# bcgsc/abyss

Hardware: AMD Instinct MI355X
Metric: Mk-mers/s inserted+extended (abyss-bloom-dbg, k=64); unitig bit-exact (higher is better)
Workload: dtype u64

## Files before the change

### abyss_amd/csrc/abg_core.h

```cpp
#pragma once

#include <stdint.h>
#include <stddef.h>

#if defined(__HIPCC__)
#include <hip/hip_runtime.h>
#define ABG_HD __host__ __device__ __forceinline__
#define ABG_HDN __host__ __device__
#define ABG_HDX __host__ __device__ __attribute__((noinline))
#else
#define ABG_HD inline
#define ABG_HDN
#define ABG_HDX
#endif

namespace abg {

constexpr int MAX_NW = 6;
constexpr int MAX_HASHES = 32;
constexpr unsigned FP_TRIM = 5;

enum Dir : int { FORWARD = 0, REVERSE = 1 };
enum Sense : int { SENSE = 0, ANTISENSE = 1 };

// ... 588 lines not shown
		rh[j] = srol_back(Q[j + k - 1] ^ (j ? Q[j - 1] : 0), j);
	}
}
#if defined(__HIP_DEVICE_COMPILE__)
ABG_HD uint64_t shfl64(uint64_t v, unsigned src)
{
	return ((uint64_t)(uint32_t)__shfl((int)(v >> 32), (int)src) << 32) | (uint32_t)__shfl((int)(uint32_t)v, (int)src);
}
template <int NW>
ABG_HD void stretch_hashes_wave(const uint32_t* __restrict__ words, uint64_t woff, uint32_t qlo, uint32_t n, unsigned k,
    uint64_t& fh, uint64_t& rh)
{
	const unsigned lane = __lane_id();
	const uint32_t nb = n + k - 1;
	const uint32_t epl = (nb + 63) >> 6;
	uint64_t pf[STRETCH_EPL], pr[STRETCH_EPL];
	uint64_t af = 0, ar = 0;
	const uint32_t t0 = lane * epl, bp0 = qlo + t0;
	uint64_t two = 0;
	if (t0 < nb) {
		const uint32_t tl = t0 + epl - 1u < nb ? t0 + epl - 1u : nb - 1u;
		const uint64_t wi = woff + (bp0 >> 4);
		const uint32_t lo = words[wi];
		const uint32_t hi = ((qlo + tl) >> 4) != (bp0 >> 4) ? words[wi + 1] : 0u;
		two = (uint64_t)lo | ((uint64_t)hi << 32);
	}
#pragma unroll
	for (unsigned i = 0; i < STRETCH_EPL; i++) {
		const uint32_t t = t0 + i;
		if (i < epl && t < nb) {
			const unsigned base = (unsigned)(two >> (2u * ((bp0 & 15u) + i))) & 3u;
			af ^= srol_back(seed_of(base), t); ar ^= srol_fwd(seed_of(3u - base), t);
		}
		pf[i] = af; pr[i] = ar;
	}
	uint64_t sf = af, sr = ar;
#pragma unroll
	for (unsigned d = 1; d < 64; d <<= 1) {
		const uint64_t tf = shfl64(sf, lane >= d ? lane - d : lane), tr = shfl64(sr, lane >= d ? lane - d : lane);
		if (lane >= d) { sf ^= tf; sr ^= tr; }
	}
	sf ^= af; sr ^= ar;
#pragma unroll
	for (unsigned i = 0; i < STRETCH_EPL; i++) { pf[i] ^= sf; pr[i] ^= sr; }
	auto fetch = [&](uint32_t t, uint64_t& vf, uint64_t& vr) {
		const unsigned src = t / epl, idx = t - src * epl;
		vf = 0; vr = 0;
#pragma unroll
		for (unsigned i = 0; i < STRETCH_EPL; i++) {
			if (i >= epl) break;
			const uint64_t xf = shfl64(pf[i], src & 63u), xr = shfl64(pr[i], src & 63u);
			if (idx == i) { vf = xf; vr = xr; }
		}
	};
	const uint32_t l = lane < n ? lane : 0;
	uint64_t hf, hr, lf, lr;
	fetch(l + k - 1, hf, hr);
	fetch(l ? l - 1 : 0, lf, lr);
	if (!l) { lf = 0; lr = 0; }
	fh = srol_fwd(hf ^ lf, k - 1 + l);
	rh = srol_back(hr ^ lr, l);
}
#endif

template <int NW, class Get>
ABG_HD Vtx<NW> gather_vertex(const Params& p, bool coop, Get get)
// ... 1499 lines not shown
```

### abyss_amd/csrc/abg_engine.h

```cpp
#pragma once
#include "abg_walk.h"

#include <algorithm>
#include <chrono>
#include <cstdio>
#include <cstdlib>
#include <cstring>
#include <functional>
#include <future>
#include <string>
#include <type_traits>
#include <vector>

namespace abg {

struct Failure { int code; std::string msg; };
constexpr int FAIL_INVAL = -1, FAIL_NOMEM = -3, FAIL_INTERNAL = -4;
[[noreturn]] inline void fail_now(int code, const std::string& msg) { throw Failure{ code, msg }; }
inline std::string strf(const char* fmt, unsigned long long a = 0, unsigned long long b = 0)
{
	char buf[256];
	snprintf(buf, sizeof buf, fmt, a, b);
	return buf;
}
// ... 18 lines not shown
	uint32_t cosettle_passes = 6;
	uint32_t cosettle_log2 = 24;
	uint32_t walk_slots = 4096;
	uint32_t tb_cap = 512;
	uint32_t buf_cap = 1u << 16;
	uint64_t pool_cap = 1ull << 28;
	uint32_t rec_cap = 1u << 22;
	uint32_t wtab_log2 = 26;
	uint32_t wtab_log2_max = 31;
	uint32_t cend_log2 = 20;
	uint64_t p2_first_batch = 65536;
	uint64_t p2_max_batch = 1ull << 22;
	uint32_t p2_growth = 2;
	uint32_t p2_crowded = 1u << 18;
	uint32_t p2_starved_growth = 2;
	uint32_t p2_starved = 6144;
	uint32_t slice_filter = 0;
	bool solid_plane = true;
	uint32_t classify_slots = 65536;
	uint32_t cls_both_max_mb = 1024;
	bool cls_both = true;
	bool prefetch_classify = true;
	uint32_t memo_log2 = 0;
	bool memo = true;
	uint32_t p2_max_candidates = 1u << 18;
	uint32_t t_tags = 1024;
	uint32_t commit_incremental = 1;
	uint32_t commit_dirty_max = 4096;
	uint32_t commit_dirty_log2 = 26;
	uint32_t guide_stride = 4;
	uint32_t guide_log2_max = 31;
	bool guide_seen = true;
	bool link_duplicates = true;
	bool par_commit = true;
	bool overlap_bins = true;
	bool overlap_purity = true;
	uint32_t dist_hash_all_ranks = 2;
	uint32_t dist_route_min_ranks = 4;
	uint64_t keep_insert_scratch_bytes = 16ull << 30;
	uint64_t par_commit_max_bytes = 16ull << 30;
	int verbose = 0;
};

struct Counters {
	uint64_t solid_reads = 0, visited_reads = 0, reads_processed = 0, bases_assembled = 0,
	         contig_id = 0;
};

struct BaseCodes {
	uint8_t t[256];
	BaseCodes()
	{
		for (int i = 0; i < 256; i++) t[i] = 0xFF;
		t['A'] = t['a'] = 0; t['C'] = t['c'] = 1; t['G'] = t['g'] = 2; t['T'] = t['t'] = 3;
	}
};
template <class T>
struct NoInitAlloc : std::allocator<T> {
	template <class U> struct rebind { using other = NoInitAlloc<U>; };
	template <class U, class... A> void construct(U* p, A&&... a)
	{
		if constexpr (sizeof...(A) == 0) ::new ((void*)p) U; else ::new ((void*)p) U(std::forward<A>(a)...);
	}
};
struct HostBatch {
	std::vector<uint32_t, NoInitAlloc<uint32_t>> words;
// ... 1605 lines not shown
		env->fast = (char*)fast + a;
		env->fast_bytes = fast_bytes - a;
		env->coop = coop;
		walk_read<NW>(*env, list[i], slot);
	}
};

template <int NW>
ABG_HDN uint64_t seq_kmer_hash(const Params& p, const uint8_t* seq, uint64_t j)
{
	return scratch_hash(p, [&](unsigned i) { return (unsigned)seq[j + i]; });
}
template <int NW>
ABG_HDN uint64_t read_kmer_hash(const Params& p, const Batch& b, uint64_t r, uint32_t j)
{
	return scratch_hash(p, [&](unsigned i) { return batch_base(b, r, j + i); });
}
constexpr uint32_t PREP_RUN = 8;
ABG_HD uint64_t dup_mix(uint64_t x) { x ^= x >> 31; x *= 0xD6E8FEB86659FD93ULL; x ^= x >> 29; x *= 0x9E3779B97F4A7C15ULL; x ^= x >> 32; return x | 1; }
template <int NW>
struct FReadPrep {
	Params p; Batch b; const uint32_t* cand_read; const uint64_t* rkoff; uint64_t* rkh; uint32_t first;
	ABG_HDN void operator()(uint64_t i, uint32_t lane, uint32_t nlanes) const
	{
		uint32_t c = first + (uint32_t)i;
		uint64_t r = cand_read[c];
		uint32_t nk = b.len[r] - p.k + 1;
		uint64_t* out = rkh + rkoff[c];
		for (uint32_t j0 = lane * PREP_RUN; j0 < nk; j0 += nlanes * PREP_RUN)
			kmer_hash_run(p, [&](unsigned q) { return batch_base(b, r, q); }, j0, j0 + PREP_RUN < nk ? j0 + PREP_RUN : nk,
			    [&](uint32_t j, uint64_t h) { out[j] = h; });
	}
};
template <int NW>
struct FContigPrep {
	Params p; const uint8_t* cnt; ContigRec* recs; uint32_t first; const uint8_t* pool; uint64_t* kh;
	uint32_t with_cov;
	ABG_HDN void operator()(uint64_t i, uint32_t lane, uint32_t nlanes) const
	{
		ContigRec& rec = recs[first + i];
		const uint8_t* seq = pool + rec.seq_off;
		uint64_t* out = kh + rec.seq_off;
		uint32_t cnk = rec.len - p.k + 1;
		uint32_t cov = 0;
		uint64_t fp = 0;
		for (uint32_t j0 = lane * PREP_RUN; j0 < cnk; j0 += nlanes * PREP_RUN)
			kmer_hash_run(p, [&](unsigned q) { return (unsigned)seq[q]; }, j0, j0 + PREP_RUN < cnk ? j0 + PREP_RUN : cnk,
			    [&](uint32_t j, uint64_t h) { out[j] = h; fp += dup_mix(h); if (with_cov) cov += solid_min_count(p, cnt, h); });
		if (cov) atomic_add_u32(&rec.coverage, cov);
		if (fp) atomic_add_u64(&rec.fp, fp);
	}
};

struct FDupKeys {
	const ContigRec* recs; uint32_t k; uint64_t* key; uint32_t* val;
	ABG_HD void operator()(uint64_t i, uint32_t) const
	{
		const ContigRec& r = recs[i];
		key[i] = r.len < k + FP_TRIM - 1 ? ~0ULL - i : dup_mix(r.fp ^ ((uint64_t)r.len << 40));
		val[i] = (uint32_t)i;
	}
};
struct FDupLink {
	ContigRec* recs; const uint64_t* key; const uint32_t* val; uint64_t n; uint32_t first_new;
	ABG_HD void operator()(uint64_t q, uint32_t) const
	{
		const uint32_t me = val[q];
		if (me < first_new) return;
		const uint64_t k = key[q];
		uint64_t g = q;
		for (unsigned s = 0; s < 64 && g > 0 && key[g - 1] == k; s++) g--;
		uint32_t best = REC_END, best_cand = recs[me].cand;
		for (unsigned s = 0; s < 128 && g < n && key[g] == k; s++, g++) {
			const uint32_t o = val[g];
			if (o != me && recs[o].cand < best_cand && recs[o].len == recs[me].len && recs[o].fp == recs[me].fp) { best = o; best_cand = recs[o].cand; }
		}
		recs[me].dup_of = best;
	}
};
struct FDupVerify {
	ContigRec* recs; const uint64_t* kh; uint32_t k; uint32_t first_new;
// ... 459 lines not shown
		if (!stop) c = c0 + nchunk;
	}
	if (tid == 0) e.st->break_at = c;
	sy.barrier();
}

constexpr uint32_t T_NEVER = 0xFFFFFFFFu;
constexpr uint32_t T_TIME_BITS = 22, T_TAGS = 1u << (32 - T_TIME_BITS);
ABG_HD uint32_t t_stamp(uint32_t tag, uint32_t time) { return (tag << T_TIME_BITS) | time; }
ABG_HD uint32_t t_read(uint32_t v, uint32_t tag) { return (v >> T_TIME_BITS) == tag ? (v & ((1u << T_TIME_BITS) - 1)) : T_NEVER; }
struct ParCommit {
	Params p; Batch b;
	const uint32_t* cand_read; const uint32_t* status; const uint32_t* first_rec;
	ContigRec* recs; const uint8_t* pool; uint8_t* result;
	const uint64_t* kh; const uint64_t* rkh; const uint64_t* rkoff; const uint8_t* read_flag;
	const uint8_t* cnt8;
	uint32_t* vis32;
	uint32_t* both32 = nullptr;
	ContigArchive arc{};
	uint32_t* T;
	uint64_t* Tk;
	uint32_t* Tv;
	uint64_t Tmask;
	uint32_t tag;
	WalkTab cend;
	WalkTab tcend;
	uint32_t* off;
	uint32_t* cnt;
	uint32_t* cnt2;
	uint64_t* cnt3;
	uint8_t* active;
	uint32_t* short_list;
	VKey* short_keys;
	uint32_t* scal;
	uint32_t* nfirst;
	uint32_t* dirty; uint32_t dirty_cap;
	uint32_t* A; uint32_t A_shift;
	uint32_t c_begin, c_end, brk;
	uint64_t own_lo, own_span;
	uint8_t* part_c; uint8_t* part_r;
};
constexpr uint64_t T_KEY_EMPTY = ~0ULL;
ABG_HD uint64_t pc_T_hash(const ParCommit& e, uint64_t pos)
{
	uint64_t x = pos * 0x9E3779B97F4A7C15ULL;
	x ^= x >> 32;
	return x & e.Tmask;
}
ABG_HD uint32_t* pc_T_slot(const ParCommit& e, uint64_t pos)
{
	if (e.T) return &e.T[pos];
	uint64_t s = pc_T_hash(e, pos);
	for (;;) {
		const uint64_t cur = cas_u64(&e.Tk[s], T_KEY_EMPTY, pos);
		if (cur == T_KEY_EMPTY || cur == pos) return &e.Tv[s];
		s = (s + 1) & e.Tmask;
	}
}
ABG_HD uint32_t pc_T_get(const ParCommit& e, uint64_t pos)
{
	if (e.T) return e.T[pos];
	uint64_t s = pc_T_hash(e, pos);
	for (;;) {
		const uint64_t cur = e.Tk[s];
		if (cur == pos) return e.Tv[s];
		if (cur == T_KEY_EMPTY) return T_NEVER;
// ... 113 lines not shown
			if (!rec.ins) continue;
			const uint64_t* ch = e.kh + rec.seq_off;
			const uint32_t cnk = rec.len - e.p.k + 1;
			for (uint32_t j = lane; j < cnk; j += nlanes) {
				uint64_t h = ch[j];
				const uint32_t which = inc ? pc_dirty_mask(e, h) : ~0u;
				if (!which) continue;
				for (unsigned q = 0; q < e.p.nh; q++) {
					if (!((which >> q) & 1u)) continue;
					const uint64_t pos = pos_i(e.p, h, q);
					if (pos - e.own_lo < e.own_span) atomic_min_u32(pc_T_slot(e, pos), t_stamp(e.tag, rec.time));
				}
			}
		}
	}
};
ABG_HD void wt_upsert_min(const WalkTab& t, const VKey& key, uint64_t time)
{
	uint64_t s = wt_slot(t, key, 0);
	for (uint64_t probes = 0; probes <= t.mask; probes++, s = (s + 1) & t.mask) {
		uint64_t cur = t.hmin[s];
		if (cur == WT_EMPTY) { t.hmin[s] = key.fh; t.hmax[s] = key.rh; t.meta[s] = time; return; }
		if (cur == key.fh && t.hmax[s] == key.rh) { if (time < t.meta[s]) t.meta[s] = time; return; }
	}
}
struct FPcShortKeys {
	ParCommit e;
	ABG_HDN void operator()(uint64_t i, uint32_t) const
	{
		const ContigRec& rec = e.recs[e.short_list[i]];
		const uint8_t* seq = e.pool + rec.seq_off;
		e.short_keys[2 * i] = canonical_end_key(e.p, seq);
		e.short_keys[2 * i + 1] = canonical_end_key(e.p, seq + rec.len - e.p.k);
	}
};
struct FPcShort {
	ParCommit e; uint32_t mode;
	ABG_HDN void operator()(uint64_t, uint32_t) const
	{
		const uint32_t n = e.scal[2];
		uint32_t added = 0;
		for (uint32_t i = 0; i < n; i++) {
			const ContigRec& rec = e.recs[e.short_list[i]];
			if (!rec.ins) continue;
			if (mode == 1 && rec.cand >= e.brk) continue;
			const VKey k1 = e.short_keys[2 * i], k2 = e.short_keys[2 * i + 1];
			if (mode == 0) {
				wt_upsert_min(e.tcend, k1, rec.time);
				wt_upsert_min(e.tcend, k2, rec.time);
			} else {
				int a = wt_insert(e.cend, k1, 0, 0), b = wt_insert(e.cend, k2, 0, 0);
				added += (a == WT_NEW) + (b == WT_NEW);
				if (a == WT_FULL || b == WT_FULL) e.scal[4] = 1;
			}
		}
		if (mode == 1) e.scal[3] = added;
	}
};
ABG_HD bool pc_end_before(const ParCommit& e, const VKey& key, uint32_t time)
{
	if (wt_find(e.cend, key, 0) != WT_EMPTY) return true;
	uint64_t s = wt_find(e.tcend, key, 0);
	return s != WT_EMPTY && e.tcend.meta[s] < (uint64_t)time;
}
template <class E>
ABG_HD bool pc_owns_no_unset_bit(const E& e, const ContigRec& rec, uint32_t lane, uint32_t nlanes, bool owned_only)
// ... 1759 lines not shown
		e.nfirst = nfirst;
		const bool incremental = cfg_.commit_incremental && (cfg_.commit_incremental > 1 || !t_hashed()) && !part && cfg_.commit_dirty_max > 0 && nrec > 0;
		uint32_t* dirty_buf = nullptr;
		e.dirty = nullptr; e.dirty_cap = 0; e.A = nullptr; e.A_shift = 0;
		if (incremental) {
			e.dirty_cap = (uint32_t)std::min<uint64_t>(std::min(cfg_.commit_dirty_max, 8192u), std::max(nrec, 1u));
			dirty_buf = (uint32_t*)be_.alloc(2ull * e.dirty_cap * 4 + 8);
			e.dirty = dirty_buf;
			if (!pcA_) {
				const uint32_t log2 = std::min(34u, std::max(10u, cfg_.commit_dirty_log2));
				pcA_bits_ = std::min<uint64_t>(m_, 1ull << log2);
				pcA_shift_ = pcA_bits_ < m_ ? 64 - log2 : 0;
				pcA_ = (uint32_t*)be_.alloc((pcA_bits_ + 31) / 32 * 4 + 4);
				be_.memset(pcA_, 0, (pcA_bits_ + 31) / 32 * 4 + 4);
			}
			e.A = pcA_; e.A_shift = pcA_shift_;
		}
		e.tcend = WalkTab{ nullptr, nullptr, nullptr, 0 };
		std::vector<uint32_t> c1(n), c2(n), off(n + 1ull);
		{ FPcCount f{ e }; be_.launch(n, f, "pc_count"); }
		be_.d2h(c1.data(), e.cnt, n * 4ull);
		off[0] = 0;
		for (uint32_t i = 0; i < n; i++) off[i + 1] = off[i] + c1[i];
		if (off[n] > (1u << T_TIME_BITS)) {
			uint32_t keep = 1;
			while (keep < n && off[keep + 1] <= (1u << T_TIME_BITS)) keep++;
			if (off[keep] > (1u << T_TIME_BITS)) fail_now(FAIL_INTERNAL, "one read produced more contigs than a commit can order");
			n = keep; c_end = c_begin + n; e.c_end = c_end; e.brk = c_end;
		}
		be_.h2d(e.off, off.data(), (n + 1ull) * 4);
		{ FPcStamp f{ e }; be_.launch(n, f, "pc_stamp"); }
		be_.d2h(scal_h, e.scal, sizeof scal_h);
		const uint32_t nshort = scal_h[2];
		e.short_keys = nullptr;
		if (nshort) {
			uint32_t log2 = 4;
			while ((1ull << log2) < 4ull * nshort) log2++;
			alloc_tab(e.tcend, log2);
			e.short_keys = (VKey*)be_.alloc(2ull * nshort * sizeof(VKey));
			FPcShortKeys f{ e };
			be_.launch(nshort, f, "pc_short_keys");
		}
		uint32_t nd = 0, nd_kmers = 0, fill = 0;
		for (uint32_t round = 0;; round++) {
			const bool inc = round && incremental && t_tag_ != 0 && nd <= e.dirty_cap && (uint64_t)nd_kmers * p_.nh * 8 <= pcA_bits_;
			const uint32_t* list = dirty_buf ? dirty_buf + (size_t)fill * e.dirty_cap : nullptr;
			if (!inc) {
				if (t_tag_ == 0) {
					if (e.T) be_.memset(e.T, 0xFF, m_ * 4ull);
					else be_.memset(e.Tv, 0xFF, 4ull << Tlog2_);
					t_tag_ = std::min<uint32_t>(cfg_.t_tags, T_TAGS) - 1;
				}
				e.tag = --t_tag_;
			} else { FPcDirty f{ e, list, 0u }; be_.launch_wave(nd, f, "pc_timemin"); }
			if (dirty_buf) { fill ^= 1; e.dirty = dirty_buf + (size_t)fill * e.dirty_cap; }
			if (nshort) {
				be_.memset(e.tcend.hmin, 0xFF, (e.tcend.mask + 1) * 8);
				FPcShort f{ e, 0 };
				be_.launch(1, f, "pc_short");
			}
			be_.memset(e.scal, 0, 4);
			be_.memset(e.scal + 5, 0, 8);
			if (round && !part && cfg_.link_duplicates) { FPcSnapshot f{ e }; be_.launch(n, f, "pc_stamp"); }
			{ FPcTimeMin f{ e, inc ? 1u : 0u }; be_.launch_wave(n, f, "pc_timemin"); }
			if (inc) { FPcDirty f{ e, list, 1u }; be_.launch_wave(nd, f, "pc_timemin"); }
			if (part) {
				be_.memset(part_buf, 1, (uint64_t)n0 + nrec);
				{ FPcDecideA f{ e }; be_.launch_wave(n, f, "pc_decide"); }
				c_all_reduce(part_buf, (uint64_t)n0 + nrec, DT_U8, OP_MIN);
				{ FPcDecideB f{ e }; be_.launch_wave(n, f, "pc_decide"); }
				c_all_reduce(part_c, n, DT_U8, OP_MAX);
				{ FPcDecideC f{ e }; be_.launch(n, f, "pc_decide"); }
			} else { FPcDecide f{ e }; be_.launch_wave(n, f, "pc_decide"); }
			be_.d2h(scal_h, e.scal, sizeof scal_h);
			stats_.commit_rounds++;
			if (inc) stats_.commit_rounds_incremental++;
			nd = scal_h[5]; nd_kmers = scal_h[6];
			stats_.commit_dirty_records += nd;
			if (!scal_h[0]) break;
		}
		{ FPcBreak f{ e }; be_.launch(n, f, "pc_break"); }
		be_.d2h(scal_h, e.scal, sizeof scal_h);
		const uint32_t brk = std::min(scal_h[1], c_end);
		e.brk = brk;
		if (sliced_) {
			ParCommit ea = e; ea.cnt8 = nullptr;
			{ FPcApply f{ ea }; be_.launch_wave(n, f, "pc_apply"); }
			const uint64_t ext = g_pool_ + 64;
			uint8_t* kmin = (uint8_t*)be_.alloc(ext);
			be_.memset(kmin, 0xFF, ext);
			{ FPcCover f{ e, kmin, 0u }; be_.launch_wave(n, f, "pc_cover"); }
			c_all_reduce(kmin, g_pool_, DT_U8, OP_MIN);
			{ FPcCover f{ e, kmin, 1u }; be_.launch_wave(n, f, "pc_cover"); }
			be_.free(kmin);
		} else { FPcApply f{ e }; be_.launch_wave(n, f, "pc_apply"); }
		if (nshort) { FPcShort f{ e, 1 }; be_.launch(1, f, "pc_short"); }
		std::vector<uint64_t> c3(n);
		std::vector<uint8_t> act(n);
		be_.d2h(c1.data(), e.cnt, n * 4ull);
		be_.d2h(c2.data(), e.cnt2, n * 4ull);
		be_.d2h(c3.data(), e.cnt3, n * 8ull);
		be_.d2h(act.data(), e.active, n);
		be_.d2h(scal_h, e.scal, sizeof scal_h);
		if (scal_h[4]) fail_now(FAIL_INTERNAL, "contigEndKmers table overflowed");
		uint32_t orec = 0; uint64_t oid = 0, bases = 0, visited = 0;
		for (uint32_t i = 0; i < n && c_begin + i < brk; i++) {
			uint32_t r = c1[i], q = c2[i];
			c1[i] = orec; c2[i] = (uint32_t)oid;
			orec += r; oid += q; bases += c3[i];
			if (!act[i]) visited++;
		}
		be_.h2d(e.cnt, c1.data(), n * 4ull);
		be_.h2d(e.cnt2, c2.data(), n * 4ull);
		{ FPcWrite f{ e, order_, nord, counters_.contig_id }; be_.launch(n, f, "pc_write"); }
		nord += orec;
		be_.h2d(order_n_, &nord, 4);
		counters_.contig_id += oid;
		counters_.bases_assembled += bases;
		counters_.visited_reads += visited;
		stats_.generated += (brk - c_begin) - visited;
		cend_count_ += scal_h[3];
		if (nshort) { free_tab(e.tcend); be_.free(e.short_keys); }
		be_.free(e.off); be_.free(e.cnt); be_.free(e.cnt2); be_.free(e.cnt3); be_.free(e.active);
		be_.free(e.short_list); be_.free(e.scal);
		if (nfirst) {
			std::vector<uint32_t> nf(n);
			be_.d2h(nf.data(), nfirst, n * 4ull);
			for (uint32_t v : nf) stats_.commit_first_chunk_decided += v;
			be_.free(nfirst);
		}
		if (dirty_buf) be_.free(dirty_buf);
		if (part_buf) be_.free(part_buf);
		return brk;
	}

	void merge_walk_results(const uint32_t* list_d, uint32_t nlist, uint32_t* status_d, uint32_t* first_d, uint32_t nc)
	{
		const uint32_t R = (uint32_t)comm_.world, me = (uint32_t)comm_.rank;
		uint32_t lr = 0; uint64_t lp = 0;
		be_.d2h(&lr, rec_used_, 4);
		be_.d2h(&lp, pool_used_, 8);
		lr = std::min(lr, rec_cap_); lp = std::min<uint64_t>(lp, pool_cap_);
		std::vector<uint64_t> cnt(2 * R, 0);
		cnt[2 * me] = lr - g_rec_; cnt[2 * me + 1] = lp - g_pool_;
		host_all_reduce_sum(cnt.data(), 2 * R);
		FRecFix fx;
		fx.rbase[0] = 0; fx.pbase[0] = 0;
		for (uint32_t q = 0; q < R; q++) {
			fx.rbase[q + 1] = fx.rbase[q] + (uint32_t)cnt[2 * q];
			fx.pbase[q + 1] = fx.pbase[q] + cnt[2 * q + 1];
		}
		const uint64_t tot_rec = fx.rbase[R], tot_pool = fx.pbase[R];
		if (g_rec_ + tot_rec > rec_cap_) {
			uint32_t cap = rec_cap_;
			while (g_rec_ + tot_rec > cap) cap *= 2;
// ... 25 lines not shown
		std::vector<uint64_t> c(R), d(R);
		for (uint32_t q = 0; q < R; q++) { c[q] = cnt[2 * q] * sizeof(ContigRec); d[q] = (uint64_t)(g_rec_ + fx.rbase[q]) * sizeof(ContigRec); }
		if (tot_rec) c_all_gather_v(recs_, c.data(), d.data());
		for (uint32_t q = 0; q < R; q++) { c[q] = cnt[2 * q + 1]; d[q] = g_pool_ + fx.pbase[q]; }
		if (tot_pool) c_all_gather_v(pool_, c.data(), d.data());
		for (uint32_t q = 0; q < R; q++) { c[q] *= 8; d[q] *= 8; }
		if (tot_pool) c_all_gather_v(kh_, c.data(), d.data());
		if (tot_rec) {
			fx.recs = recs_; fx.g_rec = g_rec_; fx.world = R;
			be_.launch(tot_rec, fx, "merge_fix");
		}
		if (nlist && fx.rbase[me]) { FFirstFix f{ list_d, first_d, fx.rbase[me] }; be_.launch(nlist, f, "merge_fix"); }
		c_all_reduce(status_d, nc, DT_U32, OP_MAX);
		c_all_reduce(first_d, nc, DT_U32, OP_MIN);
		g_rec_ += (uint32_t)tot_rec; g_pool_ += tot_pool;
		be_.h2d(rec_used_, &g_rec_, 4);
		be_.h2d(pool_used_, &g_pool_, 8);
	}
	void* regrow(void* old, uint64_t old_bytes, uint64_t new_bytes)
	{
		void* n = be_.alloc(new_bytes);
		be_.d2d(n, old, old_bytes);
		be_.free(old);
		return n;
	}

	template <int NW>
	void prep_new_records(uint32_t& prepped)
	{
		uint32_t nrec = 0;
		be_.d2h(&nrec, rec_used_, 4);
		nrec = std::min(nrec, rec_cap_);
		if (nrec > prepped) {
			FContigPrep<NW> f{ p_, cnt_, recs_, prepped, pool_, kh_, use_par_commit() ? 0u : 1u };
			be_.launch_wave(nrec - prepped, f, "contig_prep");
			if (use_par_commit()) link_duplicates(prepped, nrec);
			prepped = nrec;
		}
	}
	void link_duplicates(uint32_t first_new, uint32_t nrec)
	{
		if (!cfg_.link_duplicates || dist() || nrec <= first_new || nrec < 2) return;
		uint64_t* key = (uint64_t*)be_.alloc(nrec * 16ull); uint64_t* key2 = key + nrec;
		uint32_t* val = (uint32_t*)be_.alloc(nrec * 8ull); uint32_t* val2 = val + nrec;
		{ FDupKeys f{ recs_, p_.k, key, val }; be_.launch(nrec, f, "dup_link"); }
		be_.sort_pairs_u64_u32(key, key2, val, val2, nrec);
		{ FDupLink f{ recs_, key2, val2, nrec, first_new }; be_.launch(nrec, f, "dup_link"); }
		{ FDupVerify f{ recs_, kh_, p_.k, first_new }; be_.launch_wave(nrec - first_new, f, "dup_link"); }
		be_.sync();
		be_.free(key); be_.free(val);
	}
	template <int NW>
	void prep_local_records()
	{
		uint32_t lr = 0;
		be_.d2h(&lr, rec_used_, 4);
		lr = std::min(lr, rec_cap_);
		if (lr > g_rec_) {
			FContigPrep<NW> f{ p_, cnt_, recs_, g_rec_, pool_, kh_, use_par_commit() ? 0u : 1u };
			be_.launch_wave(lr - g_rec_, f, "contig_prep");
		}
	}
	void grow_cend()
	{
		uint32_t log2 = 1;
		while ((1ull << log2) < cend_.mask + 1) log2++;
		WalkTab bigger{};
		alloc_tab(bigger, log2 + 2);
		uint32_t* failed = (uint32_t*)be_.alloc(8);
		be_.memset(failed, 0, 4);
		FRehash f{ cend_, bigger, failed };
		be_.launch(cend_.mask + 1, f, "rehash");
		uint32_t bad = 0;
		be_.d2h(&bad, failed, 4);
		be_.free(failed);
		if (bad) fail_now(FAIL_INTERNAL, "contigEndKmers rehash failed");
		free_tab(cend_);
		cend_ = bigger;
	}
	void ensure_wtab(uint64_t nwalk)
	{
		const uint64_t want = 2 * nwalk * wtab_per_walker_;
		uint32_t log2 = wtab_log2_;
		while ((1ull << log2) < want && log2 < wtab_log2_cap()) log2++;
		if (log2 == wtab_log2_) return;
		free_tab(wtab_);
		wtab_log2_ = log2;
		alloc_tab(wtab_, wtab_log2_);
		if (cfg_.verbose) fprintf(stderr, "abyss_amd: walker vertex table grown to 2^%u entries\n", wtab_log2_);
	}
	uint32_t wtab_log2_cap()
	{
		uint32_t cap = cfg_.wtab_log2_max;
		const uint64_t mem = be_.device_mem_bytes();
// ... 344 lines not shown
```

### abyss_amd/csrc/abg_host.h

```cpp
#pragma once
#include "abg_engine.h"
#include "../../include/abyss_amd.h"

#include <cctype>
#include <cmath>
#include <map>
#include <string>
#include <atomic>
#include <chrono>
#include <future>
#include <memory>
#include <thread>

namespace abg {
static_assert(FAIL_NOMEM == ABG_ENOMEM && FAIL_INTERNAL == ABG_EINTERNAL, "Failure codes are the C ABI's");


struct FContainsSolid {
	Params p; const uint64_t* h0; const uint8_t* cnt; uint8_t* out;
	ABG_HD void operator()(uint64_t t, uint32_t) const { out[t] = solid_contains(p, cnt, h0[t]) ? 1 : 0; }
};
struct FExpand {
	Params p; const uint64_t* h0; uint64_t* out;
	ABG_HD void operator()(uint64_t t, uint32_t) const
// ... 47 lines not shown
		if (p.insert_batch_kmers) cfg.insert_batch_kmers = p.insert_batch_kmers;
		if (p.claim_log2) cfg.claim_log2 = p.claim_log2;
		if (p.walk_slots) cfg.walk_slots = p.walk_slots;
		if (p.wtab_log2) cfg.wtab_log2 = p.wtab_log2;
		if (const char* e = getenv("ABG_CLAIM_LOG2")) cfg.claim_log2 = (uint32_t)atoi(e);
		if (const char* e = getenv("ABG_INSERT_BATCH")) cfg.insert_batch_kmers = strtoull(e, 0, 10);
		if (const char* e = getenv("ABG_WALK_SLOTS")) cfg.walk_slots = (uint32_t)atoi(e);
		if (const char* e = getenv("ABG_WTAB_LOG2")) cfg.wtab_log2 = (uint32_t)atoi(e);
		if (const char* e = getenv("ABG_WTAB_LOG2_MAX")) cfg.wtab_log2_max = (uint32_t)std::max<int>(atoi(e), (int)cfg.wtab_log2);
		if (const char* e = getenv("ABG_POOL_CAP")) cfg.pool_cap = std::max<uint64_t>(1024, strtoull(e, 0, 10));
		if (const char* e = getenv("ABG_REC_CAP")) cfg.rec_cap = (uint32_t)std::max(16, atoi(e));
		if (const char* e = getenv("ABG_P2_FIRST_BATCH")) cfg.p2_first_batch = strtoull(e, 0, 10);
		if (const char* e = getenv("ABG_P2_MAX_BATCH")) cfg.p2_max_batch = strtoull(e, 0, 10);
		if (const char* e = getenv("ABG_PAR_COMMIT")) cfg.par_commit = atoi(e) != 0;
		if (const char* e = getenv("ABG_T_TAGS")) cfg.t_tags = (uint32_t)std::max(2, atoi(e));
		if (const char* e = getenv("ABG_COMMIT_INCREMENTAL")) cfg.commit_incremental = (uint32_t)std::min(2, std::max(0, atoi(e)));
		if (const char* e = getenv("ABG_COMMIT_DIRTY_MAX")) cfg.commit_dirty_max = (uint32_t)std::max(0, atoi(e));
		if (const char* e = getenv("ABG_COMMIT_DIRTY_LOG2")) cfg.commit_dirty_log2 = (uint32_t)std::min(34, std::max(10, atoi(e)));
		if (const char* e = getenv("ABG_PAR_COMMIT_MAX_GB")) cfg.par_commit_max_bytes = strtoull(e, 0, 10) << 30;
		if (const char* e = getenv("ABG_COMPACT_THRESHOLD")) cfg.compact_threshold = strtoull(e, 0, 10);
		if (const char* e = getenv("ABG_TILED")) cfg.tiled_insert = atoi(e) != 0;
		if (const char* e = getenv("ABG_DIST_ROUTE_MIN")) cfg.dist_route_min_ranks = (uint32_t)atoi(e);
		if (const char* e = getenv("ABG_BENIGN")) cfg.benign_sharers = atoi(e) != 0;
		if (const char* e = getenv("ABG_CLS_ARCHIVE")) cfg.cls_archive = atoi(e) != 0;
		if (const char* e = getenv("ABG_CLS_DEBUG_SKIP")) cfg.cls_debug_skip = (uint32_t)atoi(e);
		if (const char* e = getenv("ABG_CLS_ARCHIVE_MAX_MB")) cfg.cls_archive_max_mb = (uint32_t)std::max(0, atoi(e));
		if (const char* e = getenv("ABG_SORTED_OVERFLOW")) cfg.sorted_overflow = atoi(e) != 0;
		if (const char* e = getenv("ABG_COSETTLE")) cfg.cosettle = atoi(e) != 0;
		if (const char* e = getenv("ABG_CLS_BOTH")) cfg.cls_both = atoi(e) != 0;
		if (const char* e = getenv("ABG_CLS_BOTH_MAX_MB")) cfg.cls_both_max_mb = (uint32_t)std::max(0, atoi(e));
		if (const char* e = getenv("ABG_COSETTLE_PASSES")) cfg.cosettle_passes = (uint32_t)std::max(1, atoi(e));
		if (const char* e = getenv("ABG_COSETTLE_LOG2")) cfg.cosettle_log2 = (uint32_t)std::min(25, std::max(5, atoi(e)));
		if (const char* e = getenv("ABG_LINK_DUPS")) cfg.link_duplicates = atoi(e) != 0;
		if (const char* e = getenv("ABG_OVERLAP_PURITY")) cfg.overlap_purity = atoi(e) != 0;
		if (const char* e = getenv("ABG_OVERLAP_BINS")) cfg.overlap_bins = atoi(e) != 0;
		if (const char* e = getenv("ABG_PREFETCH")) cfg.prefetch_classify = atoi(e) != 0;
		if (const char* e = getenv("ABG_ASYNC_LOAD")) cfg.async_load = atoi(e) != 0;
		if (const char* e = getenv("ABG_CLS_SLOTS")) cfg.classify_slots = (uint32_t)std::max(64, atoi(e));
		if (const char* e = getenv("ABG_SOLID_PLANE")) cfg.solid_plane = atoi(e) != 0;
		if (const char* e = getenv("ABG_MEMO")) cfg.memo = atoi(e) != 0;
		if (const char* e = getenv("ABG_P2_MAX_CANDIDATES")) cfg.p2_max_candidates = (uint32_t)std::max(1, atoi(e));
		if (const char* e = getenv("ABG_P2_STARVED_GROWTH")) cfg.p2_starved_growth = (uint32_t)std::max(2, atoi(e));
		if (const char* e = getenv("ABG_P2_STARVED")) cfg.p2_starved = (uint32_t)atoi(e);
		if (const char* e = getenv("ABG_P2_GROWTH")) cfg.p2_growth = (uint32_t)std::max(2, atoi(e));
		if (const char* e = getenv("ABG_DRAIN_THRESHOLD")) cfg.drain_threshold = (uint32_t)strtoul(e, 0, 10);
		if (const char* e = getenv("ABG_GUIDE_STRIDE")) cfg.guide_stride = (uint32_t)strtoul(e, 0, 10);
		if (const char* e = getenv("ABG_GUIDE_SEEN")) cfg.guide_seen = atoi(e) != 0;
		if (const char* e = getenv("ABG_GUIDE_LOG2_MAX")) cfg.guide_log2_max = (uint32_t)std::min(36, std::max(10, atoi(e)));
		if (!be.ok()) return fail(ABG_ENODEV, be.why());
		eng = new Engine<BE>(be, cfg);
		return ABG_OK;
	}

	int load_seqs(const char* seqs, const uint64_t* off, uint64_t n) { return load_seqs_v(1, &seqs, &off, &n); }
	int load_seqs_v(uint32_t nchunks, const char* const* seqs_v, const uint64_t* const* off_v, const uint64_t* n_v)
	{
		const uint32_t k = cfg.k;
		const double t_call = std::chrono::duration<double>(std::chrono::steady_clock::now().time_since_epoch()).count();
		const uint32_t max_piece = (uint32_t)std::min<uint64_t>(1u << 20, cfg.insert_batch_kmers + k - 1);
		struct Part { uint32_t c; uint64_t a, b; };
		std::vector<Part> plan;
		std::vector<uint64_t> base(nchunks + 1, 0);
		for (uint32_t c = 0; c < nchunks; c++) {
			base[c + 1] = base[c] + n_v[c];
			if (!n_v[c]) continue;
			const std::vector<uint64_t> cut = split_reads(off_v[c], n_v[c]);
// ... 735 lines not shown
```

Before: 1639.

## Chunk contig prep across waves and parallelize short-contig end insertion

Contig hashing now splits each record into fixed-size chunks of k-mers, handed out as work items after a count, prefix-sum and fill step. Each wave hashes its chunk with a wave-cooperative prefix-XOR rolling hash, so one long contig no longer serializes a single wave. Separately, the single-thread short-contig end-key insertion is replaced by sorting the keys and processing each key group in parallel with CAS-based table puts. The new path adds allocations, a sort, a host sync and more launches, and it relies on the parallel grouping reproducing the serial minimum-time semantics.

New measurement: 1656, median of 5. 1.0% higher.

```diff
diff --git a/abyss_amd/csrc/abg_core.h b/abyss_amd/csrc/abg_core.h
--- a/abyss_amd/csrc/abg_core.h
+++ b/abyss_amd/csrc/abg_core.h
@@ -644,6 +644,50 @@
 			const unsigned base = (unsigned)(two >> (2u * ((bp0 & 15u) + i))) & 3u;
 			af ^= srol_back(seed_of(base), t); ar ^= srol_fwd(seed_of(3u - base), t);
 		}
+		pf[i] = af; pr[i] = ar;
+	}
+	uint64_t sf = af, sr = ar;
+#pragma unroll
+	for (unsigned d = 1; d < 64; d <<= 1) {
+		const uint64_t tf = shfl64(sf, lane >= d ? lane - d : lane), tr = shfl64(sr, lane >= d ? lane - d : lane);
+		if (lane >= d) { sf ^= tf; sr ^= tr; }
+	}
+	sf ^= af; sr ^= ar;
+#pragma unroll
+	for (unsigned i = 0; i < STRETCH_EPL; i++) { pf[i] ^= sf; pr[i] ^= sr; }
+	auto fetch = [&](uint32_t t, uint64_t& vf, uint64_t& vr) {
+		const unsigned src = t / epl, idx = t - src * epl;
+		vf = 0; vr = 0;
+#pragma unroll
+		for (unsigned i = 0; i < STRETCH_EPL; i++) {
+			if (i >= epl) break;
+			const uint64_t xf = shfl64(pf[i], src & 63u), xr = shfl64(pr[i], src & 63u);
+			if (idx == i) { vf = xf; vr = xr; }
+		}
+	};
+	const uint32_t l = lane < n ? lane : 0;
+	uint64_t hf, hr, lf, lr;
+	fetch(l + k - 1, hf, hr);
+	fetch(l ? l - 1 : 0, lf, lr);
+	if (!l) { lf = 0; lr = 0; }
+	fh = srol_fwd(hf ^ lf, k - 1 + l);
+	rh = srol_back(hr ^ lr, l);
+}
+ABG_HD void stretch_hashes_bytes_wave(const uint8_t* __restrict__ seq, uint32_t n, unsigned k, uint64_t& fh, uint64_t& rh)
+{
+	const unsigned lane = __lane_id();
+	const uint32_t nb = n + k - 1;
+	const uint32_t epl = (nb + 63) >> 6;
+	const uint32_t t0 = lane * epl;
+	unsigned base[STRETCH_EPL];
+#pragma unroll
+	for (unsigned i = 0; i < STRETCH_EPL; i++) base[i] = (i < epl && t0 + i < nb) ? (unsigned)seq[t0 + i] : 0u;
+	uint64_t pf[STRETCH_EPL], pr[STRETCH_EPL];
+	uint64_t af = 0, ar = 0;
+#pragma unroll
+	for (unsigned i = 0; i < STRETCH_EPL; i++) {
+		const uint32_t t = t0 + i;
+		if (i < epl && t < nb) { af ^= srol_back(seed_of(base[i] & 3u), t); ar ^= srol_fwd(seed_of(3u - (base[i] & 3u)), t); }
 		pf[i] = af; pr[i] = ar;
 	}
 	uint64_t sf = af, sr = ar;
diff --git a/abyss_amd/csrc/abg_engine.h b/abyss_amd/csrc/abg_engine.h
--- a/abyss_amd/csrc/abg_engine.h
+++ b/abyss_amd/csrc/abg_engine.h
@@ -74,6 +74,8 @@
 	uint32_t guide_log2_max = 31;
 	bool guide_seen = true;
 	bool link_duplicates = true;
+	bool prep_coop = true;
+	bool pc_short_par = true;
 	bool par_commit = true;
 	bool overlap_bins = true;
 	bool overlap_purity = true;
@@ -1745,21 +1747,54 @@
 			    [&](uint32_t j, uint64_t h) { out[j] = h; });
 	}
 };
+constexpr uint32_t PREP_CHUNK = 512;
+ABG_HD uint32_t prep_chunks(const ContigRec& r, uint32_t k) { return r.len < k ? 0u : (r.len - k + 1 + PREP_CHUNK - 1) / PREP_CHUNK; }
+struct FPrepCount {
+	const ContigRec* recs; uint32_t first, k; uint64_t* cum;
+	ABG_HD void operator()(uint64_t i, uint32_t) const { cum[i] = prep_chunks(recs[first + i], k); }
+};
+struct FPrepItems {
+	const ContigRec* recs; uint32_t first, k; const uint64_t* cum; uint64_t* items;
+	ABG_HD void operator()(uint64_t i, uint32_t) const
+	{
+		const uint32_t n = prep_chunks(recs[first + i], k);
+		uint64_t* to = items + (cum[i] - n);
+		for (uint32_t c = 0; c < n; c++) to[c] = (i << 32) | c;
+	}
+};
 template <int NW>
 struct FContigPrep {
 	Params p; const uint8_t* cnt; ContigRec* recs; uint32_t first; const uint8_t* pool; uint64_t* kh;
 	uint32_t with_cov;
+	const uint64_t* items;
 	ABG_HDN void operator()(uint64_t i, uint32_t lane, uint32_t nlanes) const
 	{
-		ContigRec& rec = recs[first + i];
+		uint64_t ri = i;
+		uint32_t c0 = 0;
+		if (items) { const uint64_t it = items[i]; ri = it >> 32; c0 = (uint32_t)it * PREP_CHUNK; }
+		ContigRec& rec = recs[first + ri];
 		const uint8_t* seq = pool + rec.seq_off;
 		uint64_t* out = kh + rec.seq_off;
-		uint32_t cnk = rec.len - p.k + 1;
+		const uint32_t cnk = rec.len - p.k + 1;
+		const uint32_t c1 = items && c0 + PREP_CHUNK < cnk ? c0 + PREP_CHUNK : cnk;
 		uint32_t cov = 0;
 		uint64_t fp = 0;
-		for (uint32_t j0 = lane * PREP_RUN; j0 < cnk; j0 += nlanes * PREP_RUN)
-			kmer_hash_run(p, [&](unsigned q) { return (unsigned)seq[q]; }, j0, j0 + PREP_RUN < cnk ? j0 + PREP_RUN : cnk,
-			    [&](uint32_t j, uint64_t h) { out[j] = h; fp += dup_mix(h); if (with_cov) cov += solid_min_count(p, cnt, h); });
+		auto put = [&](uint32_t j, uint64_t h) { out[j] = h; fp += dup_mix(h); if (with_cov) cov += solid_min_count(p, cnt, h); };
+		bool done = false;
+#if defined(__HIP_DEVICE_COMPILE__)
+		if (items && !p.mask && nlanes == 64) {
+			for (uint32_t s = c0; s < c1; s += 64) {
+				const uint32_t n = c1 - s < 64 ? c1 - s : 64;
+				uint64_t fh, rh;
+				stretch_hashes_bytes_wave(seq + s, n, p.k, fh, rh);
+				if (lane < n) put(s + lane, rh < fh ? rh : fh);
+			}
+			done = true;
+		}
+#endif
+		if (!done)
+			for (uint32_t j0 = c0 + lane * PREP_RUN; j0 < c1; j0 += nlanes * PREP_RUN)
+				kmer_hash_run(p, [&](unsigned q) { return (unsigned)seq[q]; }, j0, j0 + PREP_RUN < c1 ? j0 + PREP_RUN : c1, put);
 		if (cov) atomic_add_u32(&rec.coverage, cov);
 		if (fp) atomic_add_u64(&rec.fp, fp);
 	}
@@ -2285,6 +2320,8 @@
 	uint8_t* active;
 	uint32_t* short_list;
 	VKey* short_keys;
+	uint64_t* short_sk;
+	uint32_t* short_sv;
 	uint32_t* scal;
 	uint32_t* nfirst;
 	uint32_t* dirty; uint32_t dirty_cap;
@@ -2464,6 +2501,51 @@
 		const uint8_t* seq = e.pool + rec.seq_off;
 		e.short_keys[2 * i] = canonical_end_key(e.p, seq);
 		e.short_keys[2 * i + 1] = canonical_end_key(e.p, seq + rec.len - e.p.k);
+		if (e.short_sk)
+			for (uint32_t q = 2 * (uint32_t)i; q < 2 * (uint32_t)i + 2; q++) { e.short_sk[q] = e.short_keys[q].fh; e.short_sv[q] = q; }
+	}
+};
+ABG_HD bool wt_put_new(const WalkTab& t, const VKey& key, uint64_t time)
+{
+	uint64_t s = wt_slot(t, key, 0);
+	for (uint64_t probes = 0; probes <= t.mask; probes++, s = (s + 1) & t.mask)
+		if (cas_u64(&t.hmin[s], WT_EMPTY, key.fh) == WT_EMPTY) { t.hmax[s] = key.rh; t.meta[s] = time; return true; }
+	return false;
+}
+struct FPcShortPar {
+	ParCommit e; uint32_t mode;
+	ABG_HDN void operator()(uint64_t q, uint32_t) const
+	{
+		const uint64_t n2 = 2ull * e.scal[2];
+		const uint64_t* sk = e.short_sk + n2;
+		const uint32_t* sv = e.short_sv + n2;
+		const uint64_t fh = sk[q];
+		if (q && sk[q - 1] == fh) return;
+		auto enter = [&](const VKey& key, uint64_t from) {
+			bool any = false, other = false;
+			uint32_t tmin = 0xFFFFFFFFu;
+			for (uint64_t r = from; r < n2 && sk[r] == fh; r++) {
+				if (e.short_keys[sv[r]].rh != key.rh) { other = true; continue; }
+				const ContigRec& rec = e.recs[e.short_list[sv[r] >> 1]];
+				if (!rec.ins || (mode == 1 && rec.cand >= e.brk)) continue;
+				any = true;
+				tmin = rec.time < tmin ? rec.time : tmin;
+			}
+			if (any && mode == 0) wt_put_new(e.tcend, key, tmin);
+			else if (any) {
+				const int w = wt_insert(e.cend, key, 0, 0);
+				if (w == WT_NEW) atomic_add_u32(&e.scal[3], 1u);
+				if (w == WT_FULL) e.scal[4] = 1;
+			}
+			return other;
+		};
+		if (!enter(e.short_keys[sv[q]], q)) return;
+		for (uint64_t a = q + 1; a < n2 && sk[a] == fh; a++) {
+			const VKey key = e.short_keys[sv[a]];
+			bool first = true;
+			for (uint64_t r = q; r < a; r++) first = first && e.short_keys[sv[r]].rh != key.rh;
+			if (first) enter(key, a);
+		}
 	}
 };
 struct FPcShort {
@@ -4289,14 +4371,17 @@
 		{ FPcStamp f{ e }; be_.launch(n, f, "pc_stamp"); }
 		be_.d2h(scal_h, e.scal, sizeof scal_h);
 		const uint32_t nshort = scal_h[2];
-		e.short_keys = nullptr;
+		e.short_keys = nullptr; e.short_sk = nullptr; e.short_sv = nullptr;
+		const bool short_par = cfg_.pc_short_par && !part;
 		if (nshort) {
 			uint32_t log2 = 4;
 			while ((1ull << log2) < 4ull * nshort) log2++;
 			alloc_tab(e.tcend, log2);
 			e.short_keys = (VKey*)be_.alloc(2ull * nshort * sizeof(VKey));
+			if (short_par) { e.short_sk = (uint64_t*)be_.alloc(4ull * nshort * 8); e.short_sv = (uint32_t*)be_.alloc(4ull * nshort * 4); }
 			FPcShortKeys f{ e };
 			be_.launch(nshort, f, "pc_short_keys");
+			if (short_par) be_.sort_pairs_u64_u32(e.short_sk, e.short_sk + 2ull * nshort, e.short_sv, e.short_sv + 2ull * nshort, 2ull * nshort);
 		}
 		uint32_t nd = 0, nd_kmers = 0, fill = 0;
 		for (uint32_t round = 0;; round++) {
@@ -4313,8 +4398,8 @@
 			if (dirty_buf) { fill ^= 1; e.dirty = dirty_buf + (size_t)fill * e.dirty_cap; }
 			if (nshort) {
 				be_.memset(e.tcend.hmin, 0xFF, (e.tcend.mask + 1) * 8);
-				FPcShort f{ e, 0 };
-				be_.launch(1, f, "pc_short");
+				if (short_par) { FPcShortPar f{ e, 0 }; be_.launch(2ull * nshort, f, "pc_short"); }
+				else { FPcShort f{ e, 0 }; be_.launch(1, f, "pc_short"); }
 			}
 			be_.memset(e.scal, 0, 4);
 			be_.memset(e.scal + 5, 0, 8);
@@ -4351,7 +4436,8 @@
 			{ FPcCover f{ e, kmin, 1u }; be_.launch_wave(n, f, "pc_cover"); }
 			be_.free(kmin);
 		} else { FPcApply f{ e }; be_.launch_wave(n, f, "pc_apply"); }
-		if (nshort) { FPcShort f{ e, 1 }; be_.launch(1, f, "pc_short"); }
+		if (nshort && short_par) { FPcShortPar f{ e, 1 }; be_.launch(2ull * nshort, f, "pc_short"); }
+		else if (nshort) { FPcShort f{ e, 1 }; be_.launch(1, f, "pc_short"); }
 		std::vector<uint64_t> c3(n);
 		std::vector<uint8_t> act(n);
 		be_.d2h(c1.data(), e.cnt, n * 4ull);
@@ -4377,7 +4463,7 @@
 		counters_.visited_reads += visited;
 		stats_.generated += (brk - c_begin) - visited;
 		cend_count_ += scal_h[3];
-		if (nshort) { free_tab(e.tcend); be_.free(e.short_keys); }
+		if (nshort) { free_tab(e.tcend); be_.free(e.short_keys); be_.free(e.short_sk); be_.free(e.short_sv); }
 		be_.free(e.off); be_.free(e.cnt); be_.free(e.cnt2); be_.free(e.cnt3); be_.free(e.active);
 		be_.free(e.short_list); be_.free(e.scal);
 		if (nfirst) {
@@ -4469,8 +4555,7 @@
 		be_.d2h(&nrec, rec_used_, 4);
 		nrec = std::min(nrec, rec_cap_);
 		if (nrec > prepped) {
-			FContigPrep<NW> f{ p_, cnt_, recs_, prepped, pool_, kh_, use_par_commit() ? 0u : 1u };
-			be_.launch_wave(nrec - prepped, f, "contig_prep");
+			launch_contig_prep<NW>(prepped, nrec - prepped);
 			if (use_par_commit()) link_duplicates(prepped, nrec);
 			prepped = nrec;
 		}
@@ -4494,9 +4579,35 @@
 		be_.d2h(&lr, rec_used_, 4);
 		lr = std::min(lr, rec_cap_);
 		if (lr > g_rec_) {
-			FContigPrep<NW> f{ p_, cnt_, recs_, g_rec_, pool_, kh_, use_par_commit() ? 0u : 1u };
+			FContigPrep<NW> f{ p_, cnt_, recs_, g_rec_, pool_, kh_, use_par_commit() ? 0u : 1u, nullptr };
 			be_.launch_wave(lr - g_rec_, f, "contig_prep");
 		}
+	}
+	template <int NW>
+	void launch_contig_prep(uint32_t first, uint32_t n)
+	{
+		FContigPrep<NW> f{ p_, cnt_, recs_, first, pool_, kh_, use_par_commit() ? 0u : 1u, nullptr };
+		if (getenv("ABG_PREP_DEBUG")) {
+			std::vector<ContigRec> h(n);
+			be_.d2h(h.data(), recs_ + first, n * sizeof(ContigRec));
+			uint64_t tot = 0, chunks = 0; uint32_t longest = 0;
+			for (const ContigRec& r : h) { const uint32_t nk = r.len < p_.k ? 0u : r.len - p_.k + 1; tot += nk; chunks += prep_chunks(r, p_.k); longest = std::max(longest, nk); }
+			fprintf(stderr, "[prep] %u records, %llu k-mers, %llu chunks, the longest record %u k-mers\n", n, (unsigned long long)tot, (unsigned long long)chunks, longest);
+		}
+		if (!cfg_.prep_coop) { be_.launch_wave(n, f, "contig_prep"); return; }
+		uint64_t* cum = (uint64_t*)be_.alloc(n * 8ull);
+		{ FPrepCount c{ recs_, first, p_.k, cum }; be_.launch(n, c, "contig_prep"); }
+		be_.inclusive_sum_u64(cum, n);
+		uint64_t total = 0;
+		be_.d2h(&total, cum + (n - 1), 8);
+		uint64_t* items = total ? (uint64_t*)be_.alloc(total * 8ull) : nullptr;
+		if (total) {
+			{ FPrepItems c{ recs_, first, p_.k, cum, items }; be_.launch(n, c, "contig_prep"); }
+			f.items = items;
+			be_.launch_wave(total, f, "contig_prep");
+		}
+		be_.sync();
+		be_.free(items); be_.free(cum);
 	}
 	void grow_cend()
 	{
diff --git a/abyss_amd/csrc/abg_host.h b/abyss_amd/csrc/abg_host.h
--- a/abyss_amd/csrc/abg_host.h
+++ b/abyss_amd/csrc/abg_host.h
@@ -103,6 +103,9 @@
 		if (const char* e = getenv("ABG_COSETTLE_PASSES")) cfg.cosettle_passes = (uint32_t)std::max(1, atoi(e));
 		if (const char* e = getenv("ABG_COSETTLE_LOG2")) cfg.cosettle_log2 = (uint32_t)std::min(25, std::max(5, atoi(e)));
 		if (const char* e = getenv("ABG_LINK_DUPS")) cfg.link_duplicates = atoi(e) != 0;
+		if (const char* e = getenv("ABG_PREP_COOP")) cfg.prep_coop = atoi(e) != 0;
+		if (const char* e = getenv("ABG_PC_SHORT_PAR")) cfg.pc_short_par = atoi(e) != 0;
+		if (const char* e = getenv("ABG_CEND_LOG2")) cfg.cend_log2 = (uint32_t)std::min(30, std::max(4, atoi(e)));
 		if (const char* e = getenv("ABG_OVERLAP_PURITY")) cfg.overlap_purity = atoi(e) != 0;
 		if (const char* e = getenv("ABG_OVERLAP_BINS")) cfg.overlap_bins = atoi(e) != 0;
 		if (const char* e = getenv("ABG_PREFETCH")) cfg.prefetch_classify = atoi(e) != 0;
```
